# spla-tam/SplaTAM

Measured on AMD Instinct MI355X. Metric: track+map iters/sec @300k Gaussians (render+backward Mpix/s alongside), higher is better.
Workload: dtype f32; 1 GPU; B: 300000 Gaussians, 1200x680, SplaTAM tracking+mapping loop (2:3 mix), isotropic map; fused tracking iterations do not form dL/d(rgb, opacity, scale): the reference computes them, steps them with learning rate 0 and discards the optimizer after the frame (parameters after any number of iterations are identical); mapping iterations take their Adam step on gradients held in registers and do not sto; gaussians=300000, width=1200, height=680, views=8, sync_mode=auto, engine=fused, parallelism=1 process/GPU

## Files before the change

### splatam_amd/csrc/capi.hip

```cpp
#include <cstring>

#include "splat_device.h"

using namespace splat;

namespace {
int check(hipError_t e) { return e == hipSuccess ? SPLAT_OK : SPLAT_E_LAUNCH; }

bool valid_inputs(const SplatCamera *cam, const SplatGaussians *g) {
    if (!cam || !g) return false;
    if (g->P < 0 || cam->image_width <= 0 || cam->image_height <= 0) return false;
    if (cam->image_width > 65535 * SPLAT_TILE || cam->image_height > 65535 * SPLAT_TILE) return false;
    if (g->channels < 1 || g->channels > SPLAT_MAX_CHANNELS) return false;
    if (!cam->viewmatrix || !cam->projmatrix) return false;
    if (g->P > 0) {
        if (!g->means3D || !g->opacities) return false;
        if ((g->colors_precomp == nullptr) == (g->shs == nullptr)) return false;
        const bool sr = g->scales && g->rotations;
        if (sr == (g->cov3D_precomp != nullptr)) return false;
        if (g->shs) {
            if (g->channels != 3 || !cam->campos || cam->sh_degree < 0 || cam->sh_degree > 3) return false;
            if (g->sh_coeffs < (cam->sh_degree + 1) * (cam->sh_degree + 1)) return false;
        }
    }
// ... 385 lines not shown
}

int splat_map_add_new_gaussians(SplatMapStore *store, const SplatAddArgs *a, void *stream) {
    if (!valid_store(store) || !a) return SPLAT_E_INVALID;
    if (a->width < 0 || a->height < 0 || (long long)a->width * a->height > 0x7fffffffLL) return SPLAT_E_INVALID;
    if (a->mode != SPLAT_ADD_VALID_DEPTH && a->mode != SPLAT_ADD_NON_PRESENCE) return SPLAT_E_INVALID;
    if (!a->scratch || !a->im || !a->depth || a->fx == 0.f || a->fy == 0.f) return SPLAT_E_INVALID;
    if (a->mode == SPLAT_ADD_NON_PRESENCE) {
        if (!a->out6 || !a->err || !store->map.cam_unnorm_rots || !store->map.cam_trans) return SPLAT_E_INVALID;
        if (a->time_idx < 0 || a->time_idx >= store->map.num_frames) return SPLAT_E_INVALID;
    } else if (!a->w2c) {
        return SPLAT_E_INVALID;
    }
    return check(launch_map_add(*store, *a, (hipStream_t)stream));
}

int splat_map_prune(SplatMapStore *store, const SplatPruneArgs *a, void *stream) {
    if (!valid_store(store) || !a || !a->scratch) return SPLAT_E_INVALID;
    if (store->map.P > 0 && (!a->flags || !a->stage)) return SPLAT_E_INVALID;
    return check(launch_map_prune(*store, *a, (hipStream_t)stream));
}

int splat_iter_means2d_accumulate(const SplatCamera *cam, const SplatMap *map, SplatIterWorkspace *ws, float *gaccum, float *denom,
                                  float *means2D_grad, void *stream) {
    if (!cam || !map || !ws || map->P < 0 || cam->image_width <= 0 || cam->image_height <= 0) return SPLAT_E_INVALID;
    if (map->P > 0 && ((!gaccum != !denom) || (!gaccum && !means2D_grad) || !ws->accum || !ws->feat8 || !ws->dL_dout6 || !ws->st.radii || !ws->st.conic_opacity)) return SPLAT_E_INVALID;
    if (!ws->st.point_list || !ws->st.final_T || !ws->st.n_contrib || !ws->st.tile_base) return SPLAT_E_INVALID;
    return check(launch_iter_means2d_accumulate(*cam, *map, *ws, gaccum, denom, means2D_grad, (hipStream_t)stream));
}

static bool valid_densify(const SplatMapStore *store, const SplatDensifyArgs *a) {
    if (!valid_store(store) || !a || !a->flags || !a->scratch) return false;
    if (a->mode != SPLAT_DENSIFY_CLONE && a->mode != SPLAT_DENSIFY_SPLIT) return false;
    if (a->rows_with_grad < 0 || a->rows_with_grad > store->map.P) return false;
    if (a->rows_with_grad > 0 && (!store->means2D_gradient_accum || !store->denom)) return false;
    if (a->mode == SPLAT_DENSIFY_SPLIT && a->num_to_split_into < 1) return false;
    return true;
}

int splat_map_densify_select(SplatMapStore *store, const SplatDensifyArgs *a, void *stream) {
    if (!valid_densify(store, a)) return SPLAT_E_INVALID;
    return check(launch_map_densify_select(*store, *a, (hipStream_t)stream));
}

int splat_map_duplicate(SplatMapStore *store, const SplatDensifyArgs *a, void *stream) {
    if (!valid_densify(store, a)) return SPLAT_E_INVALID;
    if (a->mode == SPLAT_DENSIFY_SPLIT && !a->samples) return SPLAT_E_INVALID;
    return check(launch_map_duplicate(*store, *a, (hipStream_t)stream));
}

int splat_debug_option(int key, int value) {
    if (key == 0) { const int old = g_debug_skip_count; g_debug_skip_count = value; return old; }
    if (key == 4) { const int old = g_debug_k7_bits; g_debug_k7_bits = value; return old; }
    return -1;
}

int splat_debug_stamps(void *buffer) {
    g_debug_stamps = reinterpret_cast<long long *>(buffer);
    return SPLAT_OK;
}

int splat_selftest(int which, const void *in, void *out, int n, void *stream) {
    return check(launch_selftest(which, in, out, n, (hipStream_t)stream));
}

}

namespace {
struct LayoutWriter {
    SplatArrayInfo *out;
    int32_t max_entries, n = 0;
    size_t offset = 0;
    void add(const char *name, size_t bytes, int zero_init) {
        offset = (offset + SPLAT_SLAB_ALIGN - 1) / SPLAT_SLAB_ALIGN * SPLAT_SLAB_ALIGN;
        if (out && n < max_entries) out[n] = SplatArrayInfo{name, bytes, offset, zero_init};
        ++n;
        offset += bytes;
    }
};

void state_arrays(LayoutWriter &w, bool iter, int32_t P, int32_t width, int32_t height, int32_t sub_bins, int64_t capacity,
                  int32_t group_stride, int32_t flags) {
    const size_t T = splat_num_tiles(width, height), S = sub_bins > 1 ? (size_t)sub_bins : 1, n = (size_t)P, cap = (size_t)capacity;
    const size_t G = (size_t)(((width + SPLAT_TILE - 1) / SPLAT_TILE + SPLAT_GROUP_TILES - 1) / SPLAT_GROUP_TILES) *
                     (size_t)(((height + SPLAT_TILE - 1) / SPLAT_TILE + SPLAT_GROUP_TILES - 1) / SPLAT_GROUP_TILES);
    const size_t HW = (size_t)width * (size_t)height;
    const int z = iter ? 1 : 0;
#define NAME(f) (iter ? "st." f : f)
    w.add(NAME("depth"), 4 * n, 0);
    w.add(NAME("xy"), 8 * n, 0);
    w.add(NAME("conic_opacity"), 16 * n, 0);
    w.add(NAME("rect"), 8 * n, 0);
    w.add(NAME("radii"), 4 * n, z);
    if (flags & SPLAT_LAYOUT_SH) {
        w.add(NAME("rgb"), 12 * n, 0);
        w.add(NAME("clamped"), 3 * n, 0);
    }
    w.add(NAME("tile_count"), 4 * T * S * SPLAT_COUNTER_STRIDE, z);
    w.add(NAME("tile_base"), 4 * (T + 1), 0);
    w.add(NAME("tile_cursor"), 4 * T * S * SPLAT_COUNTER_STRIDE, 0);
    if (iter || !(flags & SPLAT_LAYOUT_GROUPS)) w.add(NAME("keys"), 8 * cap, 0);
    w.add(NAME("point_list"), 4 * cap, 0);
    if (flags & SPLAT_LAYOUT_RECS) w.add(NAME("tile_recs"), 48 * cap, 0);
    if (flags & SPLAT_LAYOUT_LONG_LISTS) {
        w.add(NAME("keys_alt"), 8 * cap, 0);
        w.add(NAME("long_items"), 4 * (cap / 1024 + T + 1), 0);
// ... 137 lines not shown
```

### splatam_amd/csrc/fused.hip

```cpp
#include "splat_device.h"

#include "fused_math.h"
#include "window_sums.h"

namespace splat {

namespace {

constexpr int kBlock = 256;
constexpr int kFlagSum = SPLAT_ITER_SUMS - 1;

struct FusedArgs {
    SplatCamera cam;
    SplatMap map;
    SplatFrameData frame;
    SplatLossConfig cfg;
    SplatIterWorkspace ws;
    float win[11];
};

__device__ __forceinline__ int c_num_tiles(int W, int H) { return ((W + kTile - 1) / kTile) * ((H + kTile - 1) / kTile); }
__device__ __forceinline__ int c_num_groups(int W, int H) {
    return (((W + kTile - 1) / kTile + SPLAT_GROUP_TILES - 1) / SPLAT_GROUP_TILES) * (((H + kTile - 1) / kTile + SPLAT_GROUP_TILES - 1) / SPLAT_GROUP_TILES);
}
// ... 476 lines not shown
        for (int j = 0; j < 4; ++j) {
            const Pixel px = GS ? depth_pixel_gs(pre[0][j], pre[3][j]) : depth_pixel(a.cfg, pre[0][j], pre[1][j], pre[2][j], pre[3][j], median);
            dout[j] = map_depth_grad(a.cfg.use_l1 != 0, a.cfg.w_depth, px.d_sign, count);
        }
        store_px4<VEC>(a.ws.dL_dout6 + 3 * HW, y0 + hr, x0 + hc, W, H, dout);
    }
}

struct PoseAdam {
    float *state;
    float beta1, beta2, eps, bc2_sqrt, ss_rot, ss_trans;
};

struct PoseAdamRegs {
    float *pp[7];
    float par[7], m[7], v[7], best;
};

__device__ __forceinline__ void pose_adam_load(const SplatMap &map, int time_idx, const PoseAdam &pa, PoseAdamRegs &r) {
#pragma unroll
    for (int k = 0; k < 7; ++k) {
        r.pp[k] = k < 4 ? map.cam_unnorm_rots + k * map.num_frames + time_idx : map.cam_trans + (k - 4) * map.num_frames + time_idx;
        r.par[k] = *r.pp[k];
        r.m[k] = pa.state[k];
        r.v[k] = pa.state[7 + k];
    }
    r.best = pa.state[14];
}

__device__ __forceinline__ void pose_adam_apply(PoseAdamRegs &r, const float *g, float loss, const PoseAdam &pa) {
    float *state = pa.state;
#pragma unroll
    for (int k = 0; k < 7; ++k)
        r.par[k] = adam_update(r.par[k], g[k], r.m[k], r.v[k], pa.beta1, pa.beta2, k < 4 ? pa.ss_rot : pa.ss_trans, pa.bc2_sqrt, pa.eps);
#pragma unroll
    for (int k = 0; k < 7; ++k) {
        *r.pp[k] = r.par[k];
        state[k] = r.m[k];
        state[7 + k] = r.v[k];
    }
    if (loss < r.best) {
        state[14] = loss;
#pragma unroll
        for (int k = 0; k < 7; ++k) state[15 + k] = r.par[k];
    }
}

__device__ __forceinline__ void pose_adam_step(const SplatMap &map, int time_idx, const float *g, float loss, const PoseAdam &pa) {
    PoseAdamRegs r;
    pose_adam_load(map, time_idx, pa, r);
    pose_adam_apply(r, g, loss, pa);
}

template <bool GS>
__global__ __launch_bounds__(256) void pose_finish_kernel(FusedArgs a, int HW, PoseAdam pa) {
    static_assert(SPLAT_ITER_SUMS * 8 == 256 && SPLAT_ITER_SUM_COPIES == 64, "thread t: sum k = t / 8, copies (t % 8) * 8 .. + 7");
    if (blockIdx.x > 0) {
        __shared__ unsigned s_order[513];
        const int T = c_num_tiles(a.cam.image_width, a.cam.image_height);
        tile_order_band(a.ws.st.tile_work, a.ws.st.tile_order, T, (T + 7) / 8, (int)blockIdx.x - 1, s_order);
        return;
    }
    __shared__ double S[SPLAT_ITER_SUMS];
    const int t = threadIdx.x, k = t >> 3, part = t & 7;
    Pose P{};
    PoseAdamRegs adam{};
    int flagged = 0, stat[4] = {0, 0, 0, 0}, skipped = 0;
    float sticky = 0.f;
    if (t == 0) {
        if (a.cfg.camera_grad) load_pose(a.map, a.frame.time_idx, P);
        if (pa.state) pose_adam_load(a.map, a.frame.time_idx, pa, adam);
#pragma unroll
        for (int k = 0; k < 4; ++k) stat[k] = a.ws.st.status[k];
        flagged = stat[SPLAT_STATUS_OVERFLOW] | stat[SPLAT_STATUS_STALE_HINT];
        sticky = a.ws.d_cam[SPLAT_REPORT_FLAG];
        skipped = reinterpret_cast<const int *>(a.ws.d_cam)[SPLAT_REPORT_SKIPPED];
    }
    double part_sum[8];
#pragma unroll
    for (int c = 0; c < 8; ++c) part_sum[c] = a.ws.sums[(size_t)(part * 8 + c) * SPLAT_ITER_SUMS + k];
    double v = 0.0;
#pragma unroll
    for (int c = 0; c < 8; ++c) {
        v += part_sum[c];
        a.ws.sums[(size_t)(part * 8 + c) * SPLAT_ITER_SUMS + k] = 0.0;
    }
    v += __shfl_xor(v, 1, 64);
    v += __shfl_xor(v, 2, 64);
    v += __shfl_xor(v, 4, 64);
    if (part == 0) S[k] = v;
    __syncthreads();
    if (t != 0) return;
    if (S[kFlagSum] != 0.0) flagged = 1;
    float *out = a.ws.d_cam;
    float dq[4] = {0.f, 0.f, 0.f, 0.f}, dt[3] = {0.f, 0.f, 0.f};
    if (a.cfg.camera_grad) {
        float sums[kPoseSums];
        for (int k = 0; k < kPoseSums; ++k) sums[k] = (float)S[8 + k];
        pose_backward(P, sums, dq, dt);
    }
    for (int k = 0; k < 4; ++k) out[SPLAT_REPORT_DROT + k] = dq[k];
    for (int k = 0; k < 3; ++k) out[SPLAT_REPORT_DTRANS + k] = dt[k];
    float loss, w_depth_term, w_im_term;
    const float l_depth = a.cfg.use_l1 ? (float)S[0] : 0.f;
    if (!GS && a.cfg.tracking) {
        w_depth_term = a.cfg.w_depth * l_depth;
        w_im_term = a.cfg.w_im * (float)S[1];
    } else {
        const float n = 3.0f * (float)HW;
        const float l_im = 0.8f * ((float)S[1] / n) + 0.2f * (1.0f - (float)S[3] / n);
        w_depth_term = a.cfg.w_depth * (a.cfg.use_l1 ? l_depth / map_depth_divisor(GS, (float)S[2], (float)HW) : 0.f);
        w_im_term = a.cfg.w_im * l_im;
    }
    loss = w_depth_term + w_im_term;
    out[SPLAT_REPORT_LOSS] = loss;
    for (int k = 0; k < 4; ++k) out[SPLAT_REPORT_SUMS + k] = (float)S[k];
    const bool gate_up = flagged != 0 || sticky != 0.f;
    if (flagged != 0) out[SPLAT_REPORT_FLAG] = 1.0f;
    out[SPLAT_REPORT_DEPTH_TERM] = w_depth_term;
    out[SPLAT_REPORT_IM_TERM] = w_im_term;
    int *outi = reinterpret_cast<int *>(out);
    for (int k = 0; k < 4; ++k) outi[SPLAT_REPORT_STATUS + k] = stat[k];
    outi[SPLAT_REPORT_FLAGGED] = flagged != 0 ? 1 : 0;
    if (gate_up) outi[SPLAT_REPORT_SKIPPED] = skipped + 1;
    if (pa.state && !gate_up) {
        float g[7];
        for (int k = 0; k < 4; ++k) g[k] = dq[k];
        for (int k = 0; k < 3; ++k) g[4 + k] = dt[k];
        pose_adam_apply(adam, g, loss, pa);
    }
}

template <bool ADAM, bool MAPGRADS, bool ISO>
__global__ __launch_bounds__(kBlock, ISO ? 5 : 4) void fused_backward_kernel(FusedArgs a, SplatAdamMap opt) {
    static_assert(MAPGRADS || !ADAM, "the Adam step consumes the map gradients");
    __shared__ double s_part[kPoseSums * (kBlock / 64)];
    const int i = blockIdx.x * kBlock + threadIdx.x;
    float pose[kPoseSums];
#pragma unroll
    for (int k = 0; k < kPoseSums; ++k) pose[k] = 0.f;
    const SplatIterWorkspace &ws = a.ws;
    constexpr bool iso = ISO;
    if (i < a.map.P) {
        CamConst c;
        load_cam(c, a.cam);
        Pose P;
        load_pose(a.map, a.frame.time_idx, P);
        const float w2c_row2[4] = {a.frame.w2c[8], a.frame.w2c[9], a.frame.w2c[10], a.frame.w2c[11]};
        constexpr bool kTrack = !MAPGRADS;
        constexpr int kRow4 = acc_row4(kTrack ? kAccTrackMask : 0xFu, !kTrack);
        static_assert(kTrack || (acc_row4(kAccTrackMask, true) == kRow4 && acc_colour_slot(false, 5) < 4 * kRow4), "one row for both mapping forms");
        float acc[SPLAT_GRAD_STRIDE];
#pragma unroll
        for (int k = 0; k < SPLAT_GRAD_STRIDE; ++k) acc[k] = 0.f;
        float4 *a4 = reinterpret_cast<float4 *>(ws.accum + (size_t)i * SPLAT_GRAD_STRIDE);
#pragma unroll
        for (int k = 0; k < kRow4; ++k) {
            const float4 v = a4[k];
            acc[4 * k] = v.x; acc[4 * k + 1] = v.y; acc[4 * k + 2] = v.z; acc[4 * k + 3] = v.w;
        }
        float p[3], u[4], logit, ls[3];
        load_gaussian(a.map, i, p, u, logit, ls);
        const float4 co = reinterpret_cast<const float4 *>(ws.st.conic_opacity)[i];
        bool gate_up = false;
        if constexpr (ADAM) gate_up = (ws.st.status[SPLAT_STATUS_OVERFLOW] | ws.st.status[SPLAT_STATUS_STALE_HINT]) != 0 || ws.d_cam[SPLAT_REPORT_FLAG] != 0.f;
#pragma unroll
        for (int k = 0; k < kRow4; ++k) a4[k] = make_float4(0.f, 0.f, 0.f, 0.f);
        const bool vis = ws.st.radii[i] > 0;
        float dp[3] = {0.f, 0.f, 0.f}, du[4] = {0.f, 0.f, 0.f, 0.f}, dlogit = 0.f, dls[3] = {0.f, 0.f, 0.f};
        float drgb[3] = {0.f, 0.f, 0.f};
        if (vis) {
            Glue G;
            glue_forward(P, w2c_row2, p, u, logit, ls, iso, G);
            float S6[6];
            cov3d_from_scale_rot(G.s, c.scale_modifier, G.rq, S6);
            float g_ndc[2], g_conic[3];
            screen_grads(acc, co.x, co.y, co.z, c.W, c.H, g_ndc, g_conic);
            float dXc[3], dS6[6], ds[3] = {0.f, 0.f, 0.f}, drq[4] = {0.f, 0.f, 0.f, 0.f};
            project_gaussian_backward(c, G.Xc, S6, g_ndc, g_conic, dXc, dS6);
            if constexpr (MAPGRADS || !ISO) cov3d_backward(G.s, c.scale_modifier, G.rq, dS6, ds, drq);
            drgb[0] = acc[acc_colour_slot(false, 0)]; drgb[1] = acc[acc_colour_slot(false, 1)]; drgb[2] = acc[acc_colour_slot(false, 2)];
            const float dz = kTrack ? acc[acc_colour_slot(true, 3)] : acc[acc_colour_slot(false, 3)] + 2.f * G.z * acc[acc_colour_slot(false, 5)];
            glue_backward(P, w2c_row2, p, iso, G, dXc, dz, kTrack ? 0.f : acc[kAccOpacity], ds, drq, dp, du, &dlogit, dls, pose);
        }
        constexpr int kWidth[5] = {3, 3, 4, 1, ISO ? 1 : 3};
        float mom1[5][4], mom2[5][4], rgb_old[3] = {0.f, 0.f, 0.f};
        if constexpr (ADAM) {
#pragma unroll
            for (int gidx = 0; gidx < 5; ++gidx)
#pragma unroll
                for (int k = 0; k < 4; ++k) {
                    const bool on = k < kWidth[gidx] && opt.grad[gidx] != nullptr;
                    mom1[gidx][k] = on ? opt.exp_avg[gidx][(size_t)i * kWidth[gidx] + k] : 0.f;
                    mom2[gidx][k] = on ? opt.exp_avg_sq[gidx][(size_t)i * kWidth[gidx] + k] : 0.f;
                }
            if (opt.grad[1]) { rgb_old[0] = a.map.rgb_colors[3 * i]; rgb_old[1] = a.map.rgb_colors[3 * i + 1]; rgb_old[2] = a.map.rgb_colors[3 * i + 2]; }
        }
        if constexpr (MAPGRADS) {
        if (a.cfg.gaussians_grad) {
            if (ws.d_means3D) { ws.d_means3D[3 * i] = dp[0]; ws.d_means3D[3 * i + 1] = dp[1]; ws.d_means3D[3 * i + 2] = dp[2]; }
            if (ws.d_unnorm_rotations)
                reinterpret_cast<float4 *>(ws.d_unnorm_rotations)[i] = iso ? make_float4(0.f, 0.f, 0.f, 0.f) : make_float4(du[0], du[1], du[2], du[3]);
        }
        if (ws.d_rgb_colors) { ws.d_rgb_colors[3 * i] = drgb[0]; ws.d_rgb_colors[3 * i + 1] = drgb[1]; ws.d_rgb_colors[3 * i + 2] = drgb[2]; }
        if (ws.d_logit_opacities) ws.d_logit_opacities[i] = dlogit;
        if (ws.d_log_scales) {
            if (iso) ws.d_log_scales[i] = dls[0];
            else { ws.d_log_scales[3 * i] = dls[0]; ws.d_log_scales[3 * i + 1] = dls[1]; ws.d_log_scales[3 * i + 2] = dls[2]; }
        }
        }
        if constexpr (ADAM) {
            const float zero4[4] = {0.f, 0.f, 0.f, 0.f};
            const float *grads[5] = {dp, drgb, iso ? zero4 : du, &dlogit, dls};
            const float *olds[5] = {p, rgb_old, u, &logit, ls};
            float *params[5] = {a.map.means3D, a.map.rgb_colors, a.map.unnorm_rotations, a.map.logit_opacities, a.map.log_scales};
#pragma unroll
            for (int gidx = 0; gidx < 5; ++gidx) {
                if (!opt.grad[gidx]) continue;
#pragma unroll
                for (int k = 0; k < 4; ++k) {
                    if (k >= kWidth[gidx]) continue;
                    float mm = mom1[gidx][k], vv = mom2[gidx][k];
                    const float gk = grads[gidx][k];
                    if ((gk == 0.f && mm == 0.f && vv == 0.f) || gate_up) continue;
                    const size_t j = (size_t)i * kWidth[gidx] + k;
                    params[gidx][j] = adam_update_c(olds[gidx][k], gk, mm, vv, opt.one_minus_beta1, opt.beta2, opt.one_minus_beta2, opt.step_size[gidx],
                                                     opt.bc2_sqrt[gidx], opt.eps);
                    opt.exp_avg[gidx][j] = mm;
                    opt.exp_avg_sq[gidx][j] = vv;
                }
            }
        }
    }
    if (ws.st.tile_stride > 0) {
        const int T = c_num_tiles(a.cam.image_width, a.cam.image_height);
        unsigned sum = 0, mx = 0;
        const int G = ws.st.group_count ? c_num_groups(a.cam.image_width, a.cam.image_height) : 0;
        for (int t = i; t < T; t += gridDim.x * kBlock) {
            const unsigned cnt = ws.st.tile_count[(size_t)t * SPLAT_COUNTER_STRIDE];
            ws.st.tile_count[(size_t)t * SPLAT_COUNTER_STRIDE] = 0;
            ws.st.tile_cursor[(size_t)t * SPLAT_COUNTER_STRIDE] = cnt;
            if (t < G) {
                group_counter_fold(ws.st, t);
            }
            sum += cnt;
            mx = max(mx, cnt);
        }
        if (blockIdx.x * kBlock < T) {
            for (int m = 32; m >= 1; m >>= 1) { sum += (unsigned)__shfl_xor((int)sum, m, 64); mx = max(mx, (unsigned)__shfl_xor((int)mx, m, 64)); }
            if ((threadIdx.x & 63) == 0 && sum) { atomicAdd((unsigned *)&ws.st.status[SPLAT_STATUS_INSTANCES], sum); atomicMax((unsigned *)&ws.st.status[SPLAT_STATUS_LONGEST], mx); }
        }
    }
    if (a.cfg.defer_finish && i == 0 && (ws.st.status[SPLAT_STATUS_OVERFLOW] | ws.st.status[SPLAT_STATUS_STALE_HINT]) != 0) atomicAdd(ws.sums + kFlagSum, 1.0);
    if (a.cfg.camera_grad) block_sums_to<kPoseSums>(sum_copy(ws.sums, SPLAT_ITER_SUMS) + 8, pose, s_part);
}

struct AdamArgs {
    SplatMap map;
    SplatAdamMap opt;
};

__global__ __launch_bounds__(kBlock) void adam_map_kernel(AdamArgs a, long long total) {
    const long long e = (long long)blockIdx.x * kBlock + threadIdx.x;
    if (e >= total) return;
    if (a.opt.gate && a.opt.gate[SPLAT_REPORT_FLAG] != 0.f) return;
    float *params[5] = {a.map.means3D, a.map.rgb_colors, a.map.unnorm_rotations, a.map.logit_opacities, a.map.log_scales};
    const int width[5] = {3, 3, 4, 1, a.map.isotropic ? 1 : 3};
    long long off = 0;
#pragma unroll
    for (int gidx = 0; gidx < 5; ++gidx) {
        const long long n = (long long)a.map.P * width[gidx];
        if (e >= off && e < off + n) {
            const float *grad = a.opt.grad[gidx];
            if (grad) {
                const long long j = e - off;
                float mm = a.opt.exp_avg[gidx][j], vv = a.opt.exp_avg_sq[gidx][j];
                const float gg = grad[j];
                if (gg == 0.f && mm == 0.f && vv == 0.f) return;
                float *p = params[gidx];
                p[j] = adam_update_c(p[j], gg, mm, vv, a.opt.one_minus_beta1, a.opt.beta2, a.opt.one_minus_beta2, a.opt.step_size[gidx],
                                     a.opt.bc2_sqrt[gidx], a.opt.eps);
                a.opt.exp_avg[gidx][j] = mm;
                a.opt.exp_avg_sq[gidx][j] = vv;
            }
        }
        off += n;
    }
}

__global__ __launch_bounds__(256) void fold_sums_kernel(double *sums) {
    static_assert(SPLAT_ITER_SUMS * 8 == 256 && SPLAT_ITER_SUM_COPIES == 64, "thread t: sum k = t / 8, copies (t % 8) * 8 .. + 7");
    const int t = threadIdx.x, k = t >> 3, part = t & 7;
    double part_sum[8];
#pragma unroll
    for (int c = 0; c < 8; ++c) part_sum[c] = sums[(size_t)(part * 8 + c) * SPLAT_ITER_SUMS + k];
    double v = 0.0;
#pragma unroll
    for (int c = 0; c < 8; ++c) {
        v += part_sum[c];
        if (part * 8 + c != 0) sums[(size_t)(part * 8 + c) * SPLAT_ITER_SUMS + k] = 0.0;
    }
    v += __shfl_xor(v, 1, 64);
    v += __shfl_xor(v, 2, 64);
    v += __shfl_xor(v, 4, 64);
    if (part == 0) sums[k] = v;
}

__global__ void adam_pose_kernel(SplatMap map, int time_idx, const float *d_cam, float *state, float beta1, float beta2,
                                 float eps, float bc2_sqrt, float ss_rot, float ss_trans) {
    if (threadIdx.x != 0 || blockIdx.x != 0) return;
    if (d_cam[SPLAT_REPORT_FLAG] != 0.f) return;
    const PoseAdam pa{state, beta1, beta2, eps, bc2_sqrt, ss_rot, ss_trans};
    pose_adam_step(map, time_idx, d_cam + SPLAT_REPORT_DROT, d_cam[SPLAT_REPORT_LOSS], pa);
}

}

hipError_t launch_depth_error_median(const float *out6, const float *depth, float *err, uint32_t *scratch, int HW, int32_t *counts,
                                     hipStream_t s);

static int num_tile_groups(const SplatCamera &cam) { return tile_groups(cam.image_width, cam.image_height); }
static bool group_binning(const SplatState &st, const SplatCamera &cam) { return group_binning(st, cam.image_width, cam.image_height); }

static int finish_blocks(const SplatState &st) {
    return (st.tile_work && st.tile_order && st.tile_row_end <= st.tile_row_begin) ? 9 : 1;
}

static IterSums iter_sums(const SplatIterWorkspace &ws, const SplatAdamMap *map_adam) {
    if (!map_adam && !ws.d_means3D && !ws.d_rgb_colors && !ws.d_unnorm_rotations && !ws.d_logit_opacities && !ws.d_log_scales) return IterSums::Track;
    return ws.d_rgb_colors || (map_adam && map_adam->grad[1]) ? IterSums::MapRgb : IterSums::Map;
}

static void launch_fused_preprocess(const FusedArgs &a, hipStream_t s) {
    const int P = a.map.P;
    if (P <= 0) return;
    const SplatState &st = a.ws.st;
    if (st.group_stride > 0)
        hipLaunchKernelGGL((fused_preprocess_kernel<2, kGroupBlock>), dim3((P + kGroupBlock - 1) / kGroupBlock), dim3(kGroupBlock),
                           sizeof(unsigned) * (size_t)num_tile_groups(a.cam), s, a);
    else if (st.order_hint && st.tile_stride > 0)
        hipLaunchKernelGGL((fused_preprocess_kernel<1, kBlock>), dim3((P + kBlock - 1) / kBlock), dim3(kBlock), 0, s, a);
    else if (st.tile_stride > 0 && !lists_sorted_by_composite(st) && P >= 8 * kDenseBlock * kDensePerThread &&
             (int)splat_num_tiles(a.cam.image_width, a.cam.image_height) <= kDenseMaxTiles)
        hipLaunchKernelGGL(fused_preprocess_dense_kernel, dim3((P + kDenseBlock * kDensePerThread - 1) / (kDenseBlock * kDensePerThread)),
                           dim3(kDenseBlock), sizeof(unsigned) * splat_num_tiles(a.cam.image_width, a.cam.image_height), s, a);
    else
        hipLaunchKernelGGL((fused_preprocess_kernel<0, kBlock>), dim3((P + kBlock - 1) / kBlock), dim3(kBlock), 0, s, a);
}

hipError_t launch_iter_loss_backward(const SplatCamera &cam, const SplatMap &map, const SplatFrameData &frame,
                                     const SplatLossConfig &cfg, SplatIterWorkspace &ws_in, hipStream_t s, const SplatPoseAdam *pose_adam,
                                     const SplatAdamMap *map_adam, int loss_mode) {
    const bool gs = loss_mode == SPLAT_LOSS_GS;
    SplatIterWorkspace ws = ws_in;
    if (!group_binning(ws.st, cam)) ws.st.group_stride = 0;
    FusedArgs a{cam, map, frame, cfg, ws, {}};
    ssim_window_host(a.win);
    const int W = cam.image_width, H = cam.image_height, HW = W * H;
    const int T = (int)splat_num_tiles(W, H);
    const int P = map.P;
    hipError_t e = hipSuccess;
    const int gblocks = (P + kBlock - 1) / kBlock;
    launch_fused_preprocess(a, s);
    if (ws.st.tile_stride == 0) {
        e = launch_tile_scan(ws.st, T, s);
        if (e != hipSuccess) return e;
    }
    SplatGaussians g{};
    g.P = P;
    g.channels = 6;
    const bool sort_in_k6 = lists_sorted_by_composite(ws.st);
    e = launch_bin_forward(cam, g, ws.st, s, !sort_in_k6);
    if (e != hipSuccess) return e;
    TrackLossEpilogue ep{frame.im, frame.depth, ws.dL_dout6, ws.sums, cfg.sil_thres, cfg.w_im, cfg.w_depth, cfg.use_sil_for_loss, cfg.use_l1};
    bool loss_done = false;
    const bool fuse_loss = cfg.tracking && !cfg.ignore_outlier_depth_loss;
    if (ws.st.tile_row_end > ws.st.tile_row_begin && !fuse_loss) return hipErrorInvalidValue;
    const bool one_kernel = fuse_loss && sort_in_k6 && cfg.fused_composite != 0;
    const IterSums sums = iter_sums(ws, map_adam);
    if (one_kernel) {
        e = launch_render_track_fused(cam, ws.feat8, ws.st, ws.out6, ws.accum, ep, cfg.fused_composite == 2, s, sums);
        if (e != hipSuccess) return e;
    } else {
        e = launch_render_forward_feat8(cam, ws.feat8, ws.st, ws.out6, sort_in_k6, s, fuse_loss ? &ep : nullptr, fuse_loss ? &loss_done : nullptr);
        if (e != hipSuccess) return e;
        if (cfg.ignore_outlier_depth_loss) {
            e = launch_depth_error_median(ws.out6, frame.depth, ws.outlier_err, ws.outlier_scratch, HW,
                                          reinterpret_cast<int32_t *>(ws.d_cam) + SPLAT_REPORT_MEDIAN - 4, s);
            if (e != hipSuccess) return e;
        }
        if (cfg.tracking && loss_done) {
        } else if (cfg.tracking) {
            if (HW % 4 == 0) {
                const int blocks = min((HW / 4 + kBlock - 1) / kBlock, 2048);
                hipLaunchKernelGGL(track_loss_kernel<4>, dim3(blocks), dim3(kBlock), 0, s, a, HW);
            } else {
                const int blocks = min((HW + kBlock - 1) / kBlock, 2048);
                hipLaunchKernelGGL(track_loss_kernel<1>, dim3(blocks), dim3(kBlock), 0, s, a, HW);
            }
        } else {
            const dim3 grid = xcd_tile_grid(W, H);
            const bool vec = (W & 3) == 0 && aligned16(ws.out6) && aligned16(frame.im) && aligned16(frame.depth) && aligned16(ws.ssim_maps) && aligned16(ws.dL_dout6);
            if (gs && vec) {
                hipLaunchKernelGGL((ssim_forward_kernel<true, true>), grid, dim3(kBlock), 0, s, a, W, H);
                hipLaunchKernelGGL((map_loss_backward_kernel<true, true>), grid, dim3(kBlock), 0, s, a, W, H);
            } else if (gs) {
                hipLaunchKernelGGL((ssim_forward_kernel<false, true>), grid, dim3(kBlock), 0, s, a, W, H);
                hipLaunchKernelGGL((map_loss_backward_kernel<false, true>), grid, dim3(kBlock), 0, s, a, W, H);
            } else if (vec) {
                hipLaunchKernelGGL((ssim_forward_kernel<true, false>), grid, dim3(kBlock), 0, s, a, W, H);
                hipLaunchKernelGGL((map_loss_backward_kernel<true, false>), grid, dim3(kBlock), 0, s, a, W, H);
            } else {
                hipLaunchKernelGGL((ssim_forward_kernel<false, false>), grid, dim3(kBlock), 0, s, a, W, H);
                hipLaunchKernelGGL((map_loss_backward_kernel<false, false>), grid, dim3(kBlock), 0, s, a, W, H);
            }
        }
        e = launch_render_backward_feat8(cam, ws.feat8, ws.st, ws.dL_dout6, ws.accum, P, false, sums, s);
        if (e != hipSuccess) return e;
    }
    PoseAdam pa{};
    if (pose_adam)
        pa = PoseAdam{pose_adam->state, pose_adam->beta1, pose_adam->beta2, pose_adam->eps, pose_adam->bc2_sqrt, pose_adam->step_size_rot,
                      pose_adam->step_size_trans};
    if (P > 0) {
        const bool iso = map.isotropic != 0;
        const bool mapgrads = sums != IterSums::Track;
        const SplatAdamMap opt = map_adam ? *map_adam : SplatAdamMap{};
        const dim3 grid(gblocks), block(kBlock);
        if (map_adam && iso) hipLaunchKernelGGL((fused_backward_kernel<true, true, true>), grid, block, 0, s, a, opt);
        else if (map_adam) hipLaunchKernelGGL((fused_backward_kernel<true, true, false>), grid, block, 0, s, a, opt);
        else if (mapgrads && iso) hipLaunchKernelGGL((fused_backward_kernel<false, true, true>), grid, block, 0, s, a, opt);
        else if (mapgrads) hipLaunchKernelGGL((fused_backward_kernel<false, true, false>), grid, block, 0, s, a, opt);
        else if (iso) hipLaunchKernelGGL((fused_backward_kernel<false, false, true>), grid, block, 0, s, a, opt);
        else hipLaunchKernelGGL((fused_backward_kernel<false, false, false>), grid, block, 0, s, a, opt);
    }
    if (gs) hipLaunchKernelGGL(pose_finish_kernel<true>, dim3(finish_blocks(ws.st)), dim3(256), 0, s, a, HW, pa);
    else if (!cfg.defer_finish) hipLaunchKernelGGL(pose_finish_kernel<false>, dim3(finish_blocks(ws.st)), dim3(256), 0, s, a, HW, pa);
    return hipGetLastError();
}

hipError_t launch_iter_finish(const SplatCamera &cam, const SplatMap &map, const SplatFrameData &frame, const SplatLossConfig &cfg,
                              SplatIterWorkspace &ws, hipStream_t s, const SplatPoseAdam *pose_adam) {
    FusedArgs a{cam, map, frame, cfg, ws, {}};
    PoseAdam pa{};
    if (pose_adam)
        pa = PoseAdam{pose_adam->state, pose_adam->beta1, pose_adam->beta2, pose_adam->eps, pose_adam->bc2_sqrt, pose_adam->step_size_rot,
                      pose_adam->step_size_trans};
    hipLaunchKernelGGL(pose_finish_kernel<false>, dim3(finish_blocks(ws.st)), dim3(256), 0, s, a, cam.image_width * cam.image_height, pa);
    return hipGetLastError();
}

hipError_t launch_fold_tile_counters(SplatState &st, int T, int G, hipStream_t s);

hipError_t launch_iter_render(const SplatCamera &cam, const SplatMap &map, const SplatFrameData &frame, SplatIterWorkspace &ws_in,
                              hipStream_t s) {
    SplatIterWorkspace ws = ws_in;
    if (!group_binning(ws.st, cam)) ws.st.group_stride = 0;
    FusedArgs a{cam, map, frame, SplatLossConfig{}, ws, {}};
    a.ws.max_2D_radius = nullptr;
    const int T = (int)splat_num_tiles(cam.image_width, cam.image_height);
    const int P = map.P;
    hipError_t e = hipSuccess;
    launch_fused_preprocess(a, s);
    if (ws.st.tile_stride == 0) {
        e = launch_tile_scan(ws.st, T, s);
        if (e != hipSuccess) return e;
    }
    SplatGaussians g{};
    g.P = P;
    g.channels = 6;
    const bool sort_in_k6 = lists_sorted_by_composite(ws.st);
    e = launch_bin_forward(cam, g, ws.st, s, !sort_in_k6);
    if (e != hipSuccess) return e;
    e = launch_render_forward_feat8(cam, ws.feat8, ws.st, ws.out6, sort_in_k6, s);
    if (e != hipSuccess) return e;
    if (ws.st.tile_stride > 0) return launch_fold_tile_counters(ws.st, T, num_tile_groups(cam), s);
// ... 68 lines not shown
```

### splatam_amd/csrc/splat_device.h

```cpp
#pragma once

#include <hip/hip_runtime.h>

#include "../../include/splat_hip.h"
#include "splat_math.h"

namespace splat {

constexpr int kWave = 64;

hipError_t launch_preprocess_forward(const SplatCamera &cam, const SplatGaussians &g, SplatState &st, hipStream_t s);
hipError_t launch_tile_count_reset(SplatState &st, int T, hipStream_t s);
hipError_t launch_tile_scan(SplatState &st, int T, hipStream_t s);
hipError_t launch_bin_forward(const SplatCamera &cam, const SplatGaussians &g, SplatState &st, hipStream_t s, bool sort = true,
                              bool counted_per_workgroup = false);

constexpr int kDenseThreads = 1024, kDenseGaussians = 4096, kDenseMaxTilesLds = 12 * 1024;
inline bool dense_exact_lists(const SplatState &st, int P, int T) {
    return st.tile_stride == 0 && st.sub_bins > 1 && P >= 8 * kDenseGaussians && T <= kDenseMaxTilesLds;
}
static_assert(4 * acc_row4((1u << SPLAT_MAX_CHANNELS) - 1u, true) <= SPLAT_GRAD_STRIDE, "every form's sums fit the accumulator row");

inline bool lists_sorted_by_composite(const SplatState &st) { return st.max_list_hint > 0 && st.max_list_hint + st.max_list_hint / 4 <= 1024; }
inline bool group_binning(const SplatState &st, int W, int H) {
// ... 11 lines not shown
hipError_t launch_same_geometry(int P, const float *oa, const float *ob, const float *sa, const float *sb, const float *ra, const float *rb,
                                int *differ, hipStream_t s);
struct TrackLossEpilogue {
    const float *im;
    const float *depth;
    float *dL_dout6;
    double *sums;
    float sil_thres, w_im, w_depth;
    int use_sil_for_loss, use_l1;
};
hipError_t launch_render_forward_feat8(const SplatCamera &cam, const float *feat8, SplatState &st, float *out6, bool sort_in_kernel,
                                       hipStream_t s, const TrackLossEpilogue *ep = nullptr, bool *ep_done = nullptr);
enum class IterSums { Track, Map, MapRgb };
hipError_t launch_render_track_fused(const SplatCamera &cam, const float *feat8, SplatState &st, float *out6, float *accum,
                                     const TrackLossEpilogue &ep, bool keep_planes, hipStream_t s, IterSums sums);
hipError_t launch_render_backward_feat8(const SplatCamera &cam, const float *feat8, const SplatState &st, const float *dL_dout6,
                                        float *accum, int P, bool zero_accum, IterSums sums, hipStream_t s);
hipError_t launch_iter_loss_backward(const SplatCamera &cam, const SplatMap &map, const SplatFrameData &frame,
                                     const SplatLossConfig &cfg, SplatIterWorkspace &ws, hipStream_t s, const SplatPoseAdam *pose_adam = nullptr,
                                     const SplatAdamMap *map_adam = nullptr, int loss_mode = SPLAT_LOSS_SPLATAM);
hipError_t launch_iter_finish(const SplatCamera &cam, const SplatMap &map, const SplatFrameData &frame, const SplatLossConfig &cfg,
                              SplatIterWorkspace &ws, hipStream_t s, const SplatPoseAdam *pose_adam);
hipError_t launch_iter_adam_map(const SplatMap &map, const SplatAdamMap &opt, hipStream_t s);
hipError_t launch_iter_fold_sums(double *sums, hipStream_t s);
hipError_t launch_iter_adam_pose(const SplatMap &map, int time_idx, const float *d_cam, float *state, float beta1, float beta2,
                                 float eps, float bc2_sqrt, float ss_rot, float ss_trans, hipStream_t s);
hipError_t launch_iter_render(const SplatCamera &cam, const SplatMap &map, const SplatFrameData &frame, SplatIterWorkspace &ws,
                              hipStream_t s);
hipError_t launch_eval_metrics(int W, int H, const float *rgb, const float *depth, const float *sil, const float *gt_im,
                               const float *gt_depth, const SplatEvalConfig &cfg, const SplatEvalWorkspace &ews, const int32_t *status,
                               double *out_row, hipStream_t s);
size_t eval_pyramid_bytes(int W, int H);
hipError_t launch_frame_prepare(int sw, int sh, const float *color, const float *depth, int dw, int dh, float *im, float *depth_out,
                                hipStream_t s);
hipError_t launch_frame_ingest(int cw, int ch, const uint8_t *rgb, int zw, int zh, const uint16_t *depth_raw, double png_depth_scale,
                               int dw, int dh, float *color_out, float *depth_out, hipStream_t s);
hipError_t launch_frame_ingest_planes(int cw, int ch, const uint8_t *rgb, int zw, int zh, const void *depth_raw, bool depth_is_float,
                                      double depth_scale, int dw, int dh, float *im, float *depth_out, hipStream_t s);
hipError_t launch_view_camera(const SplatViewArgs &v, hipStream_t s);
hipError_t launch_view_finish(const SplatViewArgs &v, hipStream_t s);
hipError_t launch_map_add(const SplatMapStore &st, const SplatAddArgs &a, hipStream_t s);
hipError_t launch_map_prune(const SplatMapStore &st, const SplatPruneArgs &a, hipStream_t s);
hipError_t launch_map_densify_select(const SplatMapStore &st, const SplatDensifyArgs &a, hipStream_t s);
hipError_t launch_map_duplicate(const SplatMapStore &st, const SplatDensifyArgs &a, hipStream_t s);
hipError_t launch_iter_means2d_accumulate(const SplatCamera &cam, const SplatMap &map, SplatIterWorkspace &ws, float *accum, float *denom,
                                          float *means2D_grad, hipStream_t s);
hipError_t launch_render_backward_rgb_only(const SplatCamera &cam, const float *feat8, const SplatState &st, const float *dL_dout6,
                                           float *accum, int P, hipStream_t s);
hipError_t launch_group_counters_restore(const SplatState &st, int G, bool live, hipStream_t s);
size_t map_scratch_words(long long n);
int map_row_floats(const SplatMapStore &st);
extern int g_debug_skip_count;
extern int g_debug_k7_bits;
extern long long *g_debug_stamps;
hipError_t launch_selftest(int which, const void *in, void *out, int n, hipStream_t s);

#if defined(__HIPCC__)

__device__ __forceinline__ void load_cam(CamConst &c, const SplatCamera &cam) {
    init_cam(c, cam.viewmatrix, cam.projmatrix, cam.image_width, cam.image_height, cam.tanfovx, cam.tanfovy,
             cam.scale_modifier);
}

__device__ __forceinline__ int lane_id() { return (int)(threadIdx.x & 63); }

__device__ __forceinline__ double *sum_copy(double *sums, int stride) { return sums + (size_t)(blockIdx.x % SPLAT_ITER_SUM_COPIES) * stride; }

template <int N, typename T = float, typename Slot>
__device__ __forceinline__ void block_sums_to(double *copy, const float (&v)[N], double *s_part , Slot slot) {
    constexpr int nw = 4;
    const int lane = threadIdx.x & 63, wave = threadIdx.x >> 6;
    T x[N];
#pragma unroll
    for (int k = 0; k < N; ++k) x[k] = (T)v[k];
    for (int m = 32; m >= 1; m >>= 1) {
#pragma unroll
        for (int k = 0; k < N; ++k) x[k] += __shfl_xor(x[k], m, 64);
    }
    if (lane == 0) {
#pragma unroll
        for (int k = 0; k < N; ++k) s_part[k * nw + wave] = (double)x[k];
    }
    __syncthreads();
    if ((int)threadIdx.x < N) {
        const double *p = s_part + threadIdx.x * nw;
        const double t = p[0] + p[1] + p[2] + p[3];
        if (t != 0.0) atomicAdd(copy + slot((int)threadIdx.x), t);
    }
}
template <int N, typename T = float>
__device__ __forceinline__ void block_sums_to(double *copy, const float (&v)[N], double *s_part) {
    block_sums_to<N, T>(copy, v, s_part, [](int k) { return k; });
}

__device__ __forceinline__ void raise_status(const SplatState &st, int k) {
    st.status[k] = 1;
    if (st.status_host) *st.status_host = 1;
}

__device__ __forceinline__ size_t sub_counter(const SplatState &st, int tile, int i) {
    const int S = st.sub_bins > 1 ? st.sub_bins : 1;
    return ((size_t)tile * S + (size_t)(i & (S - 1))) * SPLAT_COUNTER_STRIDE;
}

__device__ __forceinline__ void tile_range(const SplatState &st, int tile, unsigned &lo, int &n) {
    if (st.tile_stride > 0) {
// ... 401 lines not shown
__device__ __forceinline__ void file_group_records(const SplatState &st, unsigned *s_grp, int i, bool filed, int x0, int y0, int x1, int y1, float depth,
                                                   int ggx, int num_groups) {
    const unsigned gstride = (unsigned)st.group_stride;
    const int gx0 = x0 >> 1, gy0 = y0 >> 1;
    const int gw = filed ? ((x1 - 1) >> 1) - gx0 + 1 : 0, ng = filed ? gw * (((y1 - 1) >> 1) - gy0 + 1) : 0;
    unsigned rank[kGroupPerLane];
    const int nh = min(ng, kGroupPerLane);
#pragma unroll
    for (int t = 0; t < kGroupPerLane; ++t)
        if (t < nh) {
            const int yy = t / gw, xx = t - yy * gw;
            rank[t] = atomicAdd(&s_grp[(gy0 + yy) * ggx + gx0 + xx], 1u);
        }
    __syncthreads();
    for (int g0 = (int)threadIdx.x; g0 < num_groups; g0 += 2 * BLOCK) {
        const int g1 = g0 + BLOCK;
        const unsigned c0 = s_grp[g0], c1 = g1 < num_groups ? s_grp[g1] : 0u;
        unsigned b0 = 0u, b1 = 0u;
        if (c0) b0 = atomicAdd(&st.group_count[group_counter(g0)], c0);
        if (c1) b1 = atomicAdd(&st.group_count[group_counter(g1)], c1);
        if (c0) s_grp[g0] = b0;
        if (c1) s_grp[g1] = b1;
    }
    __syncthreads();
    const uint4 rec = make_uint4((unsigned)i, __float_as_uint(depth), (unsigned)x0 | ((unsigned)y0 << 16), (unsigned)x1 | ((unsigned)y1 << 16));
    uint4 *recs = reinterpret_cast<uint4 *>(st.group_recs);
    bool spilled = false;
    for (int t = 0; t < ng; ++t) {
        const int yy = t / gw, xx = t - yy * gw;
        const unsigned g = (unsigned)((gy0 + yy) * ggx + gx0 + xx);
        unsigned slot;
        if (t < kGroupPerLane) {
            const unsigned r = t == 0 ? rank[0] : (t == 1 ? rank[1] : (t == 2 ? rank[2] : rank[3]));
            slot = s_grp[g] + r;
        } else {
            slot = atomicAdd(&st.group_count[group_counter((int)g)], 1u);
        }
        if (slot < gstride) recs[(size_t)g * gstride + slot] = rec;
        else spilled = true;
    }
    if (spilled) raise_status(st, SPLAT_STATUS_OVERFLOW);
}

__device__ __forceinline__ unsigned wave_max_u32(unsigned v) {
    for (int m = 32; m >= 1; m >>= 1) {
        const unsigned o = (unsigned)__shfl_xor((int)v, m, 64);
        v = v > o ? v : o;
    }
    return v;
}

__device__ __forceinline__ float fast_exp2(float x) { return __builtin_amdgcn_exp2f(x); }

__device__ __forceinline__ void tile_order_band(const uint32_t *work, uint32_t *order, int T, int per_xcd, int band, unsigned *scratch) {
    unsigned *s_hist = scratch, *s_off = scratch + 256, *s_max = scratch + 512;
    const int tid = threadIdx.x;
    const int t0 = band * per_xcd, t1 = min(T, t0 + per_xcd);
    if (tid == 0) *s_max = 1u;
    s_hist[tid] = 0u;
    __syncthreads();
    unsigned mx = 0u;
    for (int t = t0 + tid; t < t1; t += 256) mx = max(mx, work[t]);
    mx = wave_max_u32(mx);
    if ((tid & 63) == 0) atomicMax(s_max, mx);
    __syncthreads();
    const float scale = 255.0f / (float)*s_max;
    for (int t = t0 + tid; t < t1; t += 256) atomicAdd(&s_hist[255 - (int)((float)work[t] * scale)], 1u);
    __syncthreads();
    if (tid < 64) {
        unsigned c[4], sum = 0u;
#pragma unroll
        for (int k = 0; k < 4; ++k) { c[k] = s_hist[4 * tid + k]; sum += c[k]; }
        unsigned incl = sum;
        for (int d = 1; d < 64; d <<= 1) {
            const unsigned o = (unsigned)__shfl_up((int)incl, d, 64);
            if (tid >= d) incl += o;
        }
        unsigned run = incl - sum;
#pragma unroll
        for (int k = 0; k < 4; ++k) { s_off[4 * tid + k] = run; run += c[k]; }
    }
    __syncthreads();
    for (int t = t0 + tid; t < t1; t += 256) {
        const unsigned pos = atomicAdd(&s_off[255 - (int)((float)work[t] * scale)], 1u);
        order[t0 + pos] = (uint32_t)t + 1u;
    }
    for (int t = max(t1, t0) + tid; t < t0 + per_xcd; t += 256) order[t] = 0xFFFFFFFFu;
}

#endif

}
```

Before: 4568 iters/s.

## Fold iteration finish into mapping backward kernel behind opt-in flag

New measurement: 4558 iters/s. Within noise of the previous version (-0.2%).

```diff
diff --git a/splatam_amd/csrc/capi.hip b/splatam_amd/csrc/capi.hip
--- a/splatam_amd/csrc/capi.hip
+++ b/splatam_amd/csrc/capi.hip
@@ -461,6 +461,7 @@
 int splat_debug_option(int key, int value) {
     if (key == 0) { const int old = g_debug_skip_count; g_debug_skip_count = value; return old; }
     if (key == 4) { const int old = g_debug_k7_bits; g_debug_k7_bits = value; return old; }
+    if (key == 5) { const int old = g_debug_mapping_close; g_debug_mapping_close = value < 0 ? -1 : (value != 0 ? 1 : 0); return old; }
     return -1;
 }
 
diff --git a/splatam_amd/csrc/fused.hip b/splatam_amd/csrc/fused.hip
--- a/splatam_amd/csrc/fused.hip
+++ b/splatam_amd/csrc/fused.hip
@@ -552,24 +552,56 @@
     pose_adam_apply(r, g, loss, pa);
 }
 
-template <bool GS>
-__global__ __launch_bounds__(256) void pose_finish_kernel(FusedArgs a, int HW, PoseAdam pa) {
+__host__ __device__ inline int finish_blocks(const SplatState &st) {
+    return (st.tile_work && st.tile_order && st.tile_row_end <= st.tile_row_begin) ? 9 : 1;
+}
+
+constexpr int kFoldBatch = 8;
+
+__device__ __forceinline__ void fold_tile_counters(const SplatState &st, int T, int G, unsigned &sum, unsigned &mx) {
+    for (unsigned t0 = threadIdx.x; t0 < (unsigned)T; t0 += 256u * kFoldBatch) {
+        unsigned cnt[kFoldBatch], grp[kFoldBatch];
+#pragma unroll
+        for (int j = 0; j < kFoldBatch; ++j) {
+            const unsigned t = t0 + 256u * j;
+            cnt[j] = t < (unsigned)T ? st.tile_count[t * SPLAT_COUNTER_STRIDE] : 0u;
+            grp[j] = t < (unsigned)G ? st.group_count[(unsigned)group_counter((int)t)] : 0u;
+        }
+#pragma unroll
+        for (int j = 0; j < kFoldBatch; ++j) {
+            const unsigned t = t0 + 256u * j;
+            if (t < (unsigned)T) {
+                st.tile_count[t * SPLAT_COUNTER_STRIDE] = 0;
+                st.tile_cursor[t * SPLAT_COUNTER_STRIDE] = cnt[j];
+            }
+            if (t < (unsigned)G) {
+                st.group_count[(unsigned)group_kept((int)t)] = grp[j];
+                st.group_count[(unsigned)group_counter((int)t)] = 0;
+            }
+            sum += cnt[j];
+            mx = max(mx, cnt[j]);
+        }
+    }
+}
+
+template <bool GS, bool POSE, bool FOLD>
+__device__ __forceinline__ void iteration_finish(const FusedArgs &a, int HW, const PoseAdam &pa, int role, double *S, unsigned *s_order) {
     static_assert(SPLAT_ITER_SUMS * 8 == 256 && SPLAT_ITER_SUM_COPIES == 64, "thread t: sum k = t / 8, copies (t % 8) * 8 .. + 7");
-    if (blockIdx.x > 0) {
-        __shared__ unsigned s_order[513];
+    if (role > 0) {
         const int T = c_num_tiles(a.cam.image_width, a.cam.image_height);
-        tile_order_band(a.ws.st.tile_work, a.ws.st.tile_order, T, (T + 7) / 8, (int)blockIdx.x - 1, s_order);
+        tile_order_band(a.ws.st.tile_work, a.ws.st.tile_order, T, (T + 7) / 8, role - 1, s_order);
         return;
     }
-    __shared__ double S[SPLAT_ITER_SUMS];
     const int t = threadIdx.x, k = t >> 3, part = t & 7;
     Pose P{};
     PoseAdamRegs adam{};
     int flagged = 0, stat[4] = {0, 0, 0, 0}, skipped = 0;
     float sticky = 0.f;
     if (t == 0) {
-        if (a.cfg.camera_grad) load_pose(a.map, a.frame.time_idx, P);
-        if (pa.state) pose_adam_load(a.map, a.frame.time_idx, pa, adam);
+        if constexpr (POSE) {
+            if (a.cfg.camera_grad) load_pose(a.map, a.frame.time_idx, P);
+            if (pa.state) pose_adam_load(a.map, a.frame.time_idx, pa, adam);
+        }
 #pragma unroll
         for (int k = 0; k < 4; ++k) stat[k] = a.ws.st.status[k];
         flagged = stat[SPLAT_STATUS_OVERFLOW] | stat[SPLAT_STATUS_STALE_HINT];
@@ -579,6 +611,15 @@
     double part_sum[8];
 #pragma unroll
     for (int c = 0; c < 8; ++c) part_sum[c] = a.ws.sums[(size_t)(part * 8 + c) * SPLAT_ITER_SUMS + k];
+    if constexpr (FOLD) {
+        if (a.ws.st.tile_stride > 0) {
+            unsigned sum = 0, mx = 0;
+            fold_tile_counters(a.ws.st, c_num_tiles(a.cam.image_width, a.cam.image_height),
+                               a.ws.st.group_count ? c_num_groups(a.cam.image_width, a.cam.image_height) : 0, sum, mx);
+            for (int m = 32; m >= 1; m >>= 1) { sum += (unsigned)__shfl_xor((int)sum, m, 64); mx = max(mx, (unsigned)__shfl_xor((int)mx, m, 64)); }
+            if ((t & 63) == 0) { s_order[t >> 6] = sum; s_order[4 + (t >> 6)] = mx; }
+        }
+    }
     double v = 0.0;
 #pragma unroll
     for (int c = 0; c < 8; ++c) {
@@ -591,13 +632,27 @@
     if (part == 0) S[k] = v;
     __syncthreads();
     if (t != 0) return;
+    if constexpr (FOLD) {
+        if (a.ws.st.tile_stride > 0) {
+            const unsigned sum = s_order[0] + s_order[1] + s_order[2] + s_order[3];
+            const unsigned mx = max(max(s_order[4], s_order[5]), max(s_order[6], s_order[7]));
+            if (sum) {
+                stat[SPLAT_STATUS_INSTANCES] = (int)((unsigned)stat[SPLAT_STATUS_INSTANCES] + sum);
+                stat[SPLAT_STATUS_LONGEST] = (int)max((unsigned)stat[SPLAT_STATUS_LONGEST], mx);
+                a.ws.st.status[SPLAT_STATUS_INSTANCES] = stat[SPLAT_STATUS_INSTANCES];
+                a.ws.st.status[SPLAT_STATUS_LONGEST] = stat[SPLAT_STATUS_LONGEST];
+            }
+        }
+    }
     if (S[kFlagSum] != 0.0) flagged = 1;
     float *out = a.ws.d_cam;
     float dq[4] = {0.f, 0.f, 0.f, 0.f}, dt[3] = {0.f, 0.f, 0.f};
-    if (a.cfg.camera_grad) {
-        float sums[kPoseSums];
-        for (int k = 0; k < kPoseSums; ++k) sums[k] = (float)S[8 + k];
-        pose_backward(P, sums, dq, dt);
+    if constexpr (POSE) {
+        if (a.cfg.camera_grad) {
+            float sums[kPoseSums];
+            for (int k = 0; k < kPoseSums; ++k) sums[k] = (float)S[8 + k];
+            pose_backward(P, sums, dq, dt);
+        }
     }
     for (int k = 0; k < 4; ++k) out[SPLAT_REPORT_DROT + k] = dq[k];
     for (int k = 0; k < 3; ++k) out[SPLAT_REPORT_DTRANS + k] = dt[k];
@@ -623,30 +678,59 @@
     for (int k = 0; k < 4; ++k) outi[SPLAT_REPORT_STATUS + k] = stat[k];
     outi[SPLAT_REPORT_FLAGGED] = flagged != 0 ? 1 : 0;
     if (gate_up) outi[SPLAT_REPORT_SKIPPED] = skipped + 1;
-    if (pa.state && !gate_up) {
-        float g[7];
-        for (int k = 0; k < 4; ++k) g[k] = dq[k];
-        for (int k = 0; k < 3; ++k) g[4 + k] = dt[k];
-        pose_adam_apply(adam, g, loss, pa);
-    }
-}
-
-template <bool ADAM, bool MAPGRADS, bool ISO>
+    if constexpr (POSE) {
+        if (pa.state && !gate_up) {
+            float g[7];
+            for (int k = 0; k < 4; ++k) g[k] = dq[k];
+            for (int k = 0; k < 3; ++k) g[4 + k] = dt[k];
+            pose_adam_apply(adam, g, loss, pa);
+        }
+    }
+}
+
+template <bool GS>
+__global__ __launch_bounds__(256) void pose_finish_kernel(FusedArgs a, int HW, PoseAdam pa) {
+    __shared__ double S[SPLAT_ITER_SUMS];
+    __shared__ unsigned s_order[513];
+    iteration_finish<GS, true, false>(a, HW, pa, (int)blockIdx.x, S, s_order);
+}
+
+template <bool ADAM, bool MAPGRADS, bool ISO, bool CLOSE = false, bool GS = false>
 __global__ __launch_bounds__(kBlock, ISO ? 5 : 4) void fused_backward_kernel(FusedArgs a, SplatAdamMap opt) {
     static_assert(MAPGRADS || !ADAM, "the Adam step consumes the map gradients");
+    static_assert(MAPGRADS || !CLOSE, "the closing form belongs to mapping");
+    static_assert(CLOSE || !GS, "the loss only matters to the closing workgroup");
+    static_assert(kBlock == 256, "iteration_finish is written for 256 threads");
     __shared__ double s_part[kPoseSums * (kBlock / 64)];
-    const int i = blockIdx.x * kBlock + threadIdx.x;
+    CamConst c;
+    Pose P;
+    float w2c_row2[4];
+    auto load_uniform = [&]() {
+        load_cam(c, a.cam);
+        load_pose(a.map, a.frame.time_idx, P);
+        for (int k = 0; k < 4; ++k) w2c_row2[k] = a.frame.w2c[8 + k];
+    };
+    unsigned block = blockIdx.x;
+    if constexpr (CLOSE) {
+        load_uniform();
+        const unsigned nfinish = (unsigned)finish_blocks(a.ws.st);
+        if (block < nfinish) {
+            __shared__ double s_sums[SPLAT_ITER_SUMS];
+            __shared__ unsigned s_order[513];
+            iteration_finish<GS, false, true>(a, a.cam.image_width * a.cam.image_height, PoseAdam{}, (int)block, s_sums, s_order);
+            return;
+        }
+        block -= nfinish;
+        __builtin_assume(block < (1u << 23));
+    }
+    const int i = block * kBlock + threadIdx.x;
     float pose[kPoseSums];
 #pragma unroll
     for (int k = 0; k < kPoseSums; ++k) pose[k] = 0.f;
     const SplatIterWorkspace &ws = a.ws;
     constexpr bool iso = ISO;
     if (i < a.map.P) {
-        CamConst c;
-        load_cam(c, a.cam);
-        Pose P;
-        load_pose(a.map, a.frame.time_idx, P);
-        const float w2c_row2[4] = {a.frame.w2c[8], a.frame.w2c[9], a.frame.w2c[10], a.frame.w2c[11]};
+        if constexpr (!CLOSE) load_uniform();
         constexpr bool kTrack = !MAPGRADS;
         constexpr int kRow4 = acc_row4(kTrack ? kAccTrackMask : 0xFu, !kTrack);
         static_assert(kTrack || (acc_row4(kAccTrackMask, true) == kRow4 && acc_colour_slot(false, 5) < 4 * kRow4), "one row for both mapping forms");
@@ -732,6 +816,7 @@
             }
         }
     }
+    if constexpr (!CLOSE)
     if (ws.st.tile_stride > 0) {
         const int T = c_num_tiles(a.cam.image_width, a.cam.image_height);
         unsigned sum = 0, mx = 0;
@@ -816,15 +901,20 @@
 
 }
 
+int g_debug_mapping_close = -1;
+static bool mapping_close() {
+    if (g_debug_mapping_close < 0) {
+        const char *e = getenv("SPLAT_MAPPING_CLOSE");
+        g_debug_mapping_close = e && e[0] != '\0' && e[0] != '0' ? 1 : 0;
+    }
+    return g_debug_mapping_close != 0;
+}
+
 hipError_t launch_depth_error_median(const float *out6, const float *depth, float *err, uint32_t *scratch, int HW, int32_t *counts,
                                      hipStream_t s);
 
 static int num_tile_groups(const SplatCamera &cam) { return tile_groups(cam.image_width, cam.image_height); }
 static bool group_binning(const SplatState &st, const SplatCamera &cam) { return group_binning(st, cam.image_width, cam.image_height); }
-
-static int finish_blocks(const SplatState &st) {
-    return (st.tile_work && st.tile_order && st.tile_row_end <= st.tile_row_begin) ? 9 : 1;
-}
 
 static IterSums iter_sums(const SplatIterWorkspace &ws, const SplatAdamMap *map_adam) {
     if (!map_adam && !ws.d_means3D && !ws.d_rgb_colors && !ws.d_unnorm_rotations && !ws.d_logit_opacities && !ws.d_log_scales) return IterSums::Track;
@@ -846,6 +936,14 @@
                            dim3(kDenseBlock), sizeof(unsigned) * splat_num_tiles(a.cam.image_width, a.cam.image_height), s, a);
     else
         hipLaunchKernelGGL((fused_preprocess_kernel<0, kBlock>), dim3((P + kBlock - 1) / kBlock), dim3(kBlock), 0, s, a);
+}
+
+template <bool GS>
+static void launch_backward_close(bool adam, bool iso, dim3 grid, dim3 block, hipStream_t s, const FusedArgs &a, const SplatAdamMap &opt) {
+    if (adam && iso) hipLaunchKernelGGL((fused_backward_kernel<true, true, true, true, GS>), grid, block, 0, s, a, opt);
+    else if (adam) hipLaunchKernelGGL((fused_backward_kernel<true, true, false, true, GS>), grid, block, 0, s, a, opt);
+    else if (iso) hipLaunchKernelGGL((fused_backward_kernel<false, true, true, true, GS>), grid, block, 0, s, a, opt);
+    else hipLaunchKernelGGL((fused_backward_kernel<false, true, false, true, GS>), grid, block, 0, s, a, opt);
 }
 
 hipError_t launch_iter_loss_backward(const SplatCamera &cam, const SplatMap &map, const SplatFrameData &frame,
@@ -922,6 +1020,16 @@
     if (pose_adam)
         pa = PoseAdam{pose_adam->state, pose_adam->beta1, pose_adam->beta2, pose_adam->eps, pose_adam->bc2_sqrt, pose_adam->step_size_rot,
                       pose_adam->step_size_trans};
+    const bool close = !cfg.tracking && !cfg.camera_grad && !cfg.defer_finish && !pa.state && P > 0 && sums != IterSums::Track &&
+                       mapping_close();
+    if (close) {
+        const bool iso = map.isotropic != 0;
+        const SplatAdamMap opt = map_adam ? *map_adam : SplatAdamMap{};
+        const dim3 grid(gblocks + finish_blocks(ws.st)), block(kBlock);
+        if (gs) launch_backward_close<true>(map_adam != nullptr, iso, grid, block, s, a, opt);
+        else launch_backward_close<false>(map_adam != nullptr, iso, grid, block, s, a, opt);
+        return hipGetLastError();
+    }
     if (P > 0) {
         const bool iso = map.isotropic != 0;
         const bool mapgrads = sums != IterSums::Track;
diff --git a/splatam_amd/csrc/splat_device.h b/splatam_amd/csrc/splat_device.h
--- a/splatam_amd/csrc/splat_device.h
+++ b/splatam_amd/csrc/splat_device.h
@@ -87,6 +87,7 @@
 int map_row_floats(const SplatMapStore &st);
 extern int g_debug_skip_count;
 extern int g_debug_k7_bits;
+extern int g_debug_mapping_close;
 extern long long *g_debug_stamps;
 hipError_t launch_selftest(int which, const void *in, void *out, int n, hipStream_t s);
 
@@ -594,20 +595,33 @@
 
 __device__ __forceinline__ float fast_exp2(float x) { return __builtin_amdgcn_exp2f(x); }
 
+constexpr int kTileOrderKeep = 4;
 __device__ __forceinline__ void tile_order_band(const uint32_t *work, uint32_t *order, int T, int per_xcd, int band, unsigned *scratch) {
     unsigned *s_hist = scratch, *s_off = scratch + 256, *s_max = scratch + 512;
     const int tid = threadIdx.x;
     const int t0 = band * per_xcd, t1 = min(T, t0 + per_xcd);
+    unsigned w[kTileOrderKeep];
+#pragma unroll
+    for (int j = 0; j < kTileOrderKeep; ++j) {
+        const int t = t0 + tid + 256 * j;
+        w[j] = t < t1 ? work[t] : 0u;
+    }
+    const int t_rest = t0 + tid + 256 * kTileOrderKeep;
     if (tid == 0) *s_max = 1u;
     s_hist[tid] = 0u;
     __syncthreads();
     unsigned mx = 0u;
-    for (int t = t0 + tid; t < t1; t += 256) mx = max(mx, work[t]);
+#pragma unroll
+    for (int j = 0; j < kTileOrderKeep; ++j) mx = max(mx, w[j]);
+    for (int t = t_rest; t < t1; t += 256) mx = max(mx, work[t]);
     mx = wave_max_u32(mx);
     if ((tid & 63) == 0) atomicMax(s_max, mx);
     __syncthreads();
     const float scale = 255.0f / (float)*s_max;
-    for (int t = t0 + tid; t < t1; t += 256) atomicAdd(&s_hist[255 - (int)((float)work[t] * scale)], 1u);
+#pragma unroll
+    for (int j = 0; j < kTileOrderKeep; ++j)
+        if (t0 + tid + 256 * j < t1) atomicAdd(&s_hist[255 - (int)((float)w[j] * scale)], 1u);
+    for (int t = t_rest; t < t1; t += 256) atomicAdd(&s_hist[255 - (int)((float)work[t] * scale)], 1u);
     __syncthreads();
     if (tid < 64) {
         unsigned c[4], sum = 0u;
@@ -623,7 +637,15 @@
         for (int k = 0; k < 4; ++k) { s_off[4 * tid + k] = run; run += c[k]; }
     }
     __syncthreads();
-    for (int t = t0 + tid; t < t1; t += 256) {
+#pragma unroll
+    for (int j = 0; j < kTileOrderKeep; ++j) {
+        const int t = t0 + tid + 256 * j;
+        if (t < t1) {
+            const unsigned pos = atomicAdd(&s_off[255 - (int)((float)w[j] * scale)], 1u);
+            order[t0 + pos] = (uint32_t)t + 1u;
+        }
+    }
+    for (int t = t_rest; t < t1; t += 256) {
         const unsigned pos = atomicAdd(&s_off[255 - (int)((float)work[t] * scale)], 1u);
         order[t0 + pos] = (uint32_t)t + 1u;
     }
```
